# vkit-x/vkit

Hardware: AMD Instinct MI355X
Metric: Mpixels/s (2048^2 RGB, geo+photo chain) (higher is better)
Workload: dtype u8; 1 GPU; C3 fused chain: camera_cubic_curve remap (level 5) + gaussian_blur(sigma=1.0) + color_shift(37) + gaussion_noise(std=10.0, the numpy stream default_rng(5000 + i) drawn on the device inside every step), states built from the configs inside every step, 2048x2048x3 uint8, batch 256 per GPU; batch_per_gpu=256, image=2048x2048x3, noise_mode=tiles, states=built on the device from the configs inside every step (vkx_camera_states_dev), lanes=1

## Files before the change

vkit_amd/csrc/chain.hip:

```cpp
#include "vkx_internal.h"

#include <stdlib.h>
#include <algorithm>
#include <memory>
#include <unordered_map>
#include <vector>

static int chain_check_items(const vkx_chain_item *items, int n_items)
{
    for (int i = 0; i < n_items; i++) {
        const vkx_chain_item &it = items[i];
        VKX_REQUIRE(it.src && it.dst && it.src_vertices && it.dst_vertices, "NULL plane in chain item");
        VKX_REQUIRE(it.sh > 0 && it.sw > 0 && it.dh > 0 && it.dw > 0, "bad shape in chain item");
        VKX_REQUIRE_PITCH(it.src_stride, (ptrdiff_t)it.sw * 3, it.sh);
        VKX_REQUIRE_PITCH(it.dst_stride, (ptrdiff_t)it.dw * 3, it.dh);
        if (it.noise && !it.noise_tiled) VKX_REQUIRE_PITCH(it.noise_stride_el, (ptrdiff_t)it.dw * 3, it.dh);
        VKX_REQUIRE_DISJOINT(it.src, it.sh, it.src_stride, (size_t)it.sw * 3, it.dst, it.dh, it.dst_stride, (size_t)it.dw * 3);
        if (it.streak_enabled) {
            VKX_REQUIRE(it.streak_thickness + it.streak_gap > 0, "streak thickness + gap must be positive");
            if (it.streak_alpha < 0.0 || it.streak_alpha > 1.0) {
                vkx_set_error("alpha=%g is invalid.", it.streak_alpha);
                return VKX_ERR_INVALID;
            }
        }
// ... 13 lines not shown
    }
    static const bool staged_only = vkx_env_on("VKX_CHAIN_STAGED", 0);
    if (!staged_only) {
        const int frc = vkx_chain_fused_try(ctx, items, n_items);
        if (frc != VKX_ERR_UNSUPPORTED) return frc;
    }
    if (int mrc = vkx_chain_consume_lattices_mark(ctx)) return mrc;
    for (int k = 0; k < 2; k++) {
        int rc = vkx_scratch_reserve(ctx, &ctx->chain[k], max_plane);
        if (rc) return rc;
    }
    for (int i = 0; i < n_items; i++) {
        const vkx_chain_item &it = items[i];
        const bool blur = it.blur_ksize > 1;
        const bool hue = it.hue_enabled != 0;
        const bool noise = it.noise != nullptr;
        const int stages_after_remap = (blur ? 1 : 0) + (hue ? 1 : 0) + (noise ? 1 : 0);
        const ptrdiff_t tmp_stride = (ptrdiff_t)it.dw * 3;
        int remaining = stages_after_remap;
        int flip = 0;
        auto next_out = [&](uint8_t *&out, ptrdiff_t &stride) {
            if (remaining == 0) { out = it.dst; stride = it.dst_stride; }
            else { out = (uint8_t *)ctx->chain[flip].ptr; stride = tmp_stride; flip ^= 1; }
        };
        uint8_t *cur = nullptr;
        ptrdiff_t cur_stride = 0;
        next_out(cur, cur_stride);
        vkx_elem e;
        e.src = it.src; e.dst = cur; e.src_stride = it.src_stride; e.dst_stride = cur_stride; e.cn = 3; e.is_f32 = 0;
        int rc = vkx_grid_remap_dev(ctx, &e, 1, it.sh, it.sw, it.src_vertices, it.dst_vertices, it.rows, it.cols, it.dh,
                                    it.dw);
        if (rc) return rc;
        if (blur) {
            remaining--;
            uint8_t *out; ptrdiff_t ostride;
            next_out(out, ostride);
            rc = vkx_gaussian_blur_u8_dev(ctx, cur, it.dh, it.dw, 3, cur_stride, it.blur_ksize, it.blur_sigma, out, ostride);
            if (rc) return rc;
            cur = out; cur_stride = ostride;
        }
        if (hue) {
            remaining--;
            uint8_t *out; ptrdiff_t ostride;
            next_out(out, ostride);
            rc = vkx_color_shift_rgb_dev(ctx, cur, it.dh, it.dw, cur_stride, it.hue_delta, out, ostride);
            if (rc) return rc;
            cur = out; cur_stride = ostride;
        }
        if (noise) {
            remaining--;
            uint8_t *out; ptrdiff_t ostride;
            next_out(out, ostride);
            const int16_t *plane = it.noise;
            ptrdiff_t plane_stride = it.noise_stride_el;
            if (it.noise_tiled) {
                const long long n = (long long)it.dh * it.dw * 3;
                if ((rc = vkx_scratch_reserve(ctx, &ctx->chain[2], (size_t)n * 2))) return rc;
                if ((rc = vkx_np_tiles_expand_dev(ctx, it.noise, n, (int16_t *)ctx->chain[2].ptr))) return rc;
                plane = (const int16_t *)ctx->chain[2].ptr;
                plane_stride = (ptrdiff_t)it.dw * 3;
            }
            rc = vkx_add_noise_i16_dev(ctx, cur, it.dh, it.dw, 3, cur_stride, plane, plane_stride, out, ostride);
            if (rc) return rc;
            cur = out; cur_stride = ostride;
        }
        if (it.streak_enabled) {
            rc = vkx_line_streak_u8_dev(ctx, it.dst, it.dh, it.dw, 3, it.dst_stride, it.streak_thickness, it.streak_gap,
                                        it.streak_dash_thickness, it.streak_dash_gap, it.streak_color, it.streak_alpha,
                                        it.streak_enable_vert, it.streak_enable_hori);
            if (rc) return rc;
        }
    }
    return VKX_OK;
}

VKX_EXPORT int vkx_chain_rgb_batch_np_dev(vkx_ctx *ctx, const vkx_chain_item *items, int n_items, const vkx_np_job *jobs, int n_jobs,
                                          vkx_np_result *results_host)
{
    VKX_REQUIRE(ctx != nullptr, "ctx is NULL");
    VKX_REQUIRE(n_items >= 0 && (n_items == 0 || items), "bad item list");
    if (n_jobs <= 0) return vkx_chain_rgb_batch_dev(ctx, items, n_items);
    int rc = vkx_np_jobs_check(jobs, n_jobs, results_host);
    if (rc) return rc;
    if ((rc = chain_check_items(items, n_items))) return rc;
    std::unordered_map<const void *, int> item_of;
    for (int i = 0; i < n_items; i++)
        if (items[i].noise && items[i].noise_tiled) item_of[(const void *)items[i].noise] = i;
    bool pipelined = (jobs[0].kind & 0xff) == VKX_NP_NORMAL_TILES;
    std::vector<int> job_item((size_t)n_jobs, -1);
    for (int k = 0; k < n_jobs && pipelined; k++) {
        auto it = item_of.find(jobs[k].dst);
        if (it == item_of.end() || (k > 0 && it->second <= job_item[k - 1])) pipelined = false;
        else job_item[k] = it->second;
    }
    static const bool staged_only = vkx_env_on("VKX_CHAIN_STAGED", 0);
    static const int chunks_env = vkx_env_int("VKX_CHAIN_CHUNKS", 0);
    const int want_chunks = chunks_env > 0 ? chunks_env : 2;
    vkx_chain_plan *raw = nullptr;
    if (pipelined && !staged_only) {
        rc = vkx_chain_plan_build(ctx, items, n_items, &raw);
        if (rc && rc != VKX_ERR_UNSUPPORTED) return rc;
    }
    if (!raw) {
        if ((rc = vkx_chain_consume_lattices_mark(ctx))) return rc;
        if ((rc = vkx_np_draw_batch_dev(ctx, jobs, n_jobs, results_host))) return rc;
        return vkx_chain_rgb_batch_dev(ctx, items, n_items);
    }
    std::unique_ptr<vkx_chain_plan, void (*)(vkx_chain_plan *)> plan(raw, vkx_chain_plan_free);
    const int n_chunks = std::max(1, std::min(want_chunks, n_jobs / 8));
    struct Chunk { int job0, njobs, item0, nitems; vkx_np_chunk *np; hipEvent_t posted; };
    std::vector<Chunk> chunks((size_t)n_chunks);
    for (int c = 0; c < n_chunks; c++) {
        Chunk &ch = chunks[c];
        ch.job0 = (int)((long long)n_jobs * c / n_chunks);
        ch.njobs = (int)((long long)n_jobs * (c + 1) / n_chunks) - ch.job0;
        ch.item0 = c == 0 ? 0 : job_item[ch.job0];
        ch.np = nullptr; ch.posted = nullptr;
    }
    for (int c = 0; c < n_chunks; c++) chunks[c].nitems = (c + 1 < n_chunks ? chunks[c + 1].item0 : n_items) - chunks[c].item0;
    struct Cleanup {
        std::vector<Chunk> &chunks;
        ~Cleanup() { for (Chunk &ch : chunks) { if (ch.np) vkx_np_chunk_free(ch.np); if (ch.posted) (void)hipEventDestroy(ch.posted); } }
    } cleanup{chunks};

    vkx_device_guard guard(ctx);
    hipStream_t main_stream = ctx->stream;
    const char *fail_env = getenv("VKX_DEBUG_FAIL_CHUNK");
    const int fail_chunk = fail_env && fail_env[0] ? atoi(fail_env) : -1;
    auto schedule = [&]() -> int {
        int rc = VKX_OK;
        hipStream_t aux = vkx_stream_by_id(ctx, VKX_STREAM_COPY_IN, &rc);
        if (rc) return rc;
        hipEvent_t setup_done = nullptr;
        if ((rc = vkx_chain_plan_setup_aside(ctx, raw, &setup_done))) return rc;
        if (setup_done) VKX_HIP(hipStreamWaitEvent(aux, setup_done, 0));
        for (int c = 0; c < n_chunks; c++) {
            Chunk &ch = chunks[c];
            if (c >= 2) VKX_HIP(hipStreamWaitEvent(main_stream, chunks[c - 2].posted, 0));
            if ((rc = vkx_np_chunk_begin(ctx, jobs + ch.job0, ch.njobs, results_host + ch.job0, c & 1, &ch.np))) return rc;
            if ((rc = vkx_stream_order(ctx, aux, main_stream))) return rc;
            ctx->stream = aux;
            rc = vkx_np_chunk_finish(ctx, ch.np);
            if (!rc) rc = vkx_chain_plan_noise_rows(ctx, raw, ch.item0, ch.nitems);
            ctx->stream = main_stream;
            if (rc) return rc;
            VKX_HIP(hipEventCreateWithFlags(&ch.posted, hipEventDisableTiming));
            VKX_HIP(hipEventRecord(ch.posted, aux));
            if (c == fail_chunk) {
                vkx_set_error("injected failure in chunk %d (VKX_DEBUG_FAIL_CHUNK)", c);
                return VKX_ERR_INVALID;
            }
        }
        if (setup_done) VKX_HIP(hipStreamWaitEvent(main_stream, setup_done, 0));
        for (int c = 0; c < n_chunks; c++) {
            Chunk &ch = chunks[c];
            VKX_HIP(hipStreamWaitEvent(main_stream, ch.posted, 0));
            if ((rc = vkx_chain_plan_tiles(ctx, raw, ch.item0, ch.nitems))) return rc;
        }
        return vkx_chain_mark_done(ctx, main_stream);
    };
    rc = schedule();
    if (rc) vkx_ctx_join_streams(ctx, main_stream);
    return rc;
}
```

vkit_amd/csrc/fused.hip:

```cpp
#include "vkx_internal.h"
#include "vkx_cell.h"
#include "vkx_color.h"

#include <float.h>
#include <memory>
#include <stdlib.h>
#include <string.h>

namespace {

constexpr int W = 64;
constexpr int RMAX = 3;
constexpr int NLDSCELL = 64;
#ifndef VKX_FUSED_NWAVES
#define VKX_FUSED_NWAVES 8
#endif
constexpr int NWAVES = VKX_FUSED_NWAVES;
constexpr int NTHREADS = 64 * NWAVES;
constexpr int ROWS_PER_WAVE = 8;
constexpr int WH = NWAVES * ROWS_PER_WAVE;
__host__ __device__ constexpr int tile_side(int R) { return (W - 2 * R) & ~3; }
__host__ __device__ constexpr int tile_height(int R) { return WH == W ? tile_side(R) : WH - 2 * R; }
#ifndef VKX_FUSED_CGROUP
#define VKX_FUSED_CGROUP 2
// ... 784 lines not shown
    const uint32_t g4 = (uint32_t)((ocx >> 2) * 12 + (ocx & 3) * 4);
    const uint32_t k3 = grouped ? g4 : (uint32_t)(ocx * 3);
    const bool nlane = ocol && !(grouped && (ocx & 3) == 3);
    constexpr bool every_lane = INTERIOR;
    const uint32_t k3n = (every_lane && !nlane) ? 0u : k3;
    const uint32_t k3b = k3n << 1;
    long long prow = (long long)(y0 + wave) * (long long)nstride + (long long)x0 * 3;
    const long long pstep = (long long)NWAVES * (long long)nstride;
    if (noise) {
#pragma unroll
        for (int i = 0; i < ROWS_PER_WAVE; i++) {
            const int cy = wave + NWAVES * i;
            const long long prow_i = prow;
            prow += pstep;
            if (!row_live(i, cy)) continue;
            const uint32_t rx = (uint32_t)__builtin_amdgcn_readlane((int)nrow.x, i);
            const uint32_t sd = (uint32_t)__builtin_amdgcn_readlane((int)nrow.y, i) | never;
            const gbytes_t rowb = nbase + 2 * (tiled ? (long long)rx : prow_i);
            uint32_t off = k3b;
            if ((sd & 0xffffu) < 3u * W) {
                asm volatile("" ::: "memory");
                off += k3n >= (sd & 0xffffu) ? (uint32_t)((int)sd >> 16) << 1 : 0u;
            }
            const gbytes_t np_ = rowb + (size_t)off;
            if (!every_lane) { nzA[i] = 0; nzB[i] = 0; }
            if (every_lane || nlane) {
                if (grouped) {
                    const unsigned long long v = *(const u64_u1 VKX_GLOBAL *)np_;
                    nzA[i] = (uint32_t)v;
                    nzB[i] = (uint32_t)(v >> 32);
                } else {
                    nzA[i] = *(const u32_u1 VKX_GLOBAL *)np_;
                    nzB[i] = *(const u16_u1 VKX_GLOBAL *)(np_ + 4);
                }
            }
        }
    }
    uint32_t wpair[RMAX + 1];
#pragma unroll
    for (int q = 0; q <= RMAX; q++) {
        const uint32_t e0 = 2 * q < K ? kq[2 * q < 2 * RMAX + 1 ? 2 * q : 0] : 0u, e1 = 2 * q + 1 < K ? kq[2 * q + 1 < 2 * RMAX + 1 ? 2 * q + 1 : 0] : 0u;
        const uint32_t o0 = (q > 0 && 2 * q - 1 < K) ? kq[q > 0 ? 2 * q - 1 : 0] : 0u, o1 = 2 * q < K ? kq[2 * q < 2 * RMAX + 1 ? 2 * q : 0] : 0u;
        wpair[q] = (wave & 1) ? (o0 | (o1 << 16)) : (e0 | (e1 << 16));
    }
    const int right4 = min(lane + 1, 63) << 2;
    const uint32_t dcol4 = (uint32_t)(x0 * 3) + g4;
    const bool streak_on = STREAK && ite.streak_on != 0;
    const int sxm = streak_on ? (x0 + ocx) % ite.streak_step : 0;
    const int sxd = streak_on ? (x0 + ocx) % ite.streak_dash_step : 0;
    uint32_t epx = 0;
    if constexpr (EMPTY) {
        int er = src[0], eg = src[1], eb = src[2];
        if (hue_on) hue_shift_px(lut->sdiv, lut->hdiv, hue_delta, er, eg, eb);
        epx = (uint32_t)er | ((uint32_t)eg << 8) | ((uint32_t)eb << 16);
    }
#pragma unroll
    for (int i = 0; i < ROWS_PER_WAVE; i++) {
        const int cy = wave + NWAVES * i;
        if (!row_live(i, cy)) continue;
        const int gy = y0 + cy;
        uint32_t P = epx;
        if constexpr (!EMPTY) {
            if (R > 0) {
                int r, g, b;
                if constexpr (INTERIOR && RC > 0) {
                    const uint32_t *pl = own + (cy & ~1) * P_ + lane;
                    uint32_t ar = 32768u, ag = 32768u, ab = 32768u;
#pragma unroll
                    for (int q = 0; q <= RC; q++) {
                        ar = dot2_u16_ks(wpair[q], pl[q * kPairPitch], ar);
                        ag = dot2_u16_ks(wpair[q], pl[q * kPairPitch + 64], ag);
                        ab = dot2_u16_ks(wpair[q], pl[q * kPairPitch + 128], ab);
                    }
                    r = (int)(ar >> 16); g = (int)(ag >> 16); b = (int)(ab >> 16);
                } else {
                    uint32_t a0 = 0, a1 = 0, a2 = 0;
#pragma unroll
                    for (int j = 0; j < 2 * RMAX + 1; j++) {
                        if (j < K) {
                            const int yy = INTERIOR ? cy + j : vkd::reflect101(gy + j - R, dh) - wy0;
                            const uint16_t *h16 = (const uint16_t *)(own + (yy & ~1) * P_ + lane) + (yy & 1);
                            a0 += __umul24(kq[j], (uint32_t)h16[0]);
                            a1 += __umul24(kq[j], (uint32_t)h16[128]);
                            a2 += __umul24(kq[j], (uint32_t)h16[256]);
                        }
                    }
                    r = (int)((a0 + 32768u) >> 16); g = (int)((a1 + 32768u) >> 16); b = (int)((a2 + 32768u) >> 16);
                }
                if (phase_limit == 20) {
                    const int yy = INTERIOR ? cy + R : vkd::reflect101(gy, dh) - wy0;
                    const uint16_t *h16 = (const uint16_t *)(own + (yy & ~1) * P_ + lane) + (yy & 1);
                    r = h16[0] >> 8; g = h16[128] >> 8; b = h16[256] >> 8;
                }
                if (hue_on) P = vkd::hue_shift_packed(lsdiv, lhdiv, lsel, hue_delta, r, g, b);
                else P = (uint32_t)r | ((uint32_t)g << 8) | ((uint32_t)b << 16);
            } else {
                P = own[(cy + R) * P_ + lane];
                if (hue_on) P = vkd::hue_shift_packed(lsdiv, lhdiv, lsel, hue_delta, (int)(P & 0xff), (int)((P >> 8) & 0xff),
                                                      (int)((P >> 16) & 0xff));
            }
        }
        if ((STREAK || !INTERIOR) && ((noise && !grouped) || (STREAK && streak_on))) {
            int r = (int)(P & 0xff), g = (int)((P >> 8) & 0xff), b = (int)((P >> 16) & 0xff);
            if (noise) {
                r = vkd::clamp_u8((int)(int16_t)(r + (int)(nzA[i] & 0xffff)));
                g = vkd::clamp_u8((int)(int16_t)(g + (int)(nzA[i] >> 16)));
                b = vkd::clamp_u8((int)(int16_t)(b + (int)(nzB[i] & 0xffff)));
            }
            if (STREAK && streak_on) {
                const int ym = gy % ite.streak_step, yd = gy % ite.streak_dash_step;
                bool mv = ite.streak_vert && sxm < ite.streak_thickness;
                bool mh = ite.streak_hori && ym < ite.streak_thickness;
                if (ite.streak_dash) {
                    if (yd < ite.streak_dash_gap) mv = false;
                    if (sxd < ite.streak_dash_gap) mh = false;
                }
                const float w1 = ite.streak_alpha, w0 = 1.0f - w1;
                int *ch[3] = {&r, &g, &b};
#pragma unroll
                for (int c = 0; c < 3; c++) {
                    int v = *ch[c];
                    const int col = ite.streak_color[c];
                    if (mv) { const float t0 = w0 * (float)v, t1 = w1 * (float)col; v = ite.streak_copy ? col : (int)(uint8_t)(t0 + t1); }
                    if (mh) { const float t0 = w0 * (float)v, t1 = w1 * (float)col; v = ite.streak_copy ? col : (int)(uint8_t)(t0 + t1); }
                    *ch[c] = v;
                }
            }
            P = (uint32_t)r | ((uint32_t)g << 8) | ((uint32_t)b << 16);
        }
        const uint32_t Pn = (uint32_t)__builtin_amdgcn_ds_bpermute(right4, (int)P);
        gdst_t drow = dst + (ptrdiff_t)gy * dstride + (ptrdiff_t)x0 * 3;
        if (ocol) {
            const int m = ocx & 3;
            if (INTERIOR || ocx < full4) {
                if (m < 3) {
                    uint32_t wv = (P >> (8 * m)) | (Pn << (24 - 8 * m));
                    if (!STREAK && noise) wv = add_noise_u8x4(wv, nzA[i], nzB[i]);
                    const uint32_t off = (uint32_t)gy * (uint32_t)dstride + dcol4;
                    *(u32_u1 VKX_GLOBAL *)(dst + (size_t)off) = wv;
                }
            } else {
                gdst_t d = drow + ocx * 3;
                d[0] = (uint8_t)P; d[1] = (uint8_t)(P >> 8); d[2] = (uint8_t)(P >> 16);
            }
        }
    }
}

template <bool STREAK>
__global__ void __launch_bounds__(NTHREADS, VKX_FUSED_WAVES_PER_EU) k_chain_fused(const ItemDev *__restrict__ items,
                                                          const vkc::CellC *__restrict__ cells,
                                                          const TileBin *__restrict__ bins, int bin_slots,
                                                          int *__restrict__ over_count, int2 *__restrict__ over_list, int over_slots,
                                                          const HsvLut *__restrict__ lut, int phase_limit)
{
    const ItemDev &it = items[blockIdx.y];
    const int rw = it.rect_w;
    const int nrect = rw * it.rect_h;
    const int per = (nrect + 7) >> 3;
    const int run = (int)((blockIdx.x + blockIdx.y) & 7), pos = (int)(blockIdx.x >> 3);
    const int rl = run * per + pos;
    if (pos >= per || rl >= nrect) return;
    if (phase_limit == 10) return;
    const int ry = __builtin_amdgcn_readfirstlane(div_small(rl, rw, __builtin_amdgcn_rcpf((float)rw)));
    const int tx = it.rect_x0 + rl - ry * rw, ty = it.rect_y0 + ry;
    const int tl = ty * it.tiles_x + tx;
    const TileBin bin = bins[(size_t)blockIdx.y * bin_slots + tl];
    const int nc = bin.rmax1 > 0 ? max(0, bin.rmax1 - bin.rmin) * max(0, bin.cmax1 - bin.cmin) : 0;
#ifdef VKX_FUSED_CENSUS
    (void)nc;
    chain_tile<1, STREAK, VKX_FUSED_CENSUS>(it, tx, ty, cells, bin, lut, phase_limit);
    return;
#endif
    if (nc == 0) chain_tile<2, STREAK>(it, tx, ty, cells, bin, lut, phase_limit);
    else if (nc <= NLDSCELL && phase_limit != 3) {
        switch (it.R) {
        case 0: chain_tile<1, STREAK, 0>(it, tx, ty, cells, bin, lut, phase_limit); break;
        case 1: chain_tile<1, STREAK, 1>(it, tx, ty, cells, bin, lut, phase_limit); break;
        case 2: chain_tile<1, STREAK, 2>(it, tx, ty, cells, bin, lut, phase_limit); break;
        default: chain_tile<1, STREAK, 3>(it, tx, ty, cells, bin, lut, phase_limit); break;
        }
    } else if (threadIdx.x == 0) {
        const int k = atomicAdd(over_count, 1);
        if (k < over_slots) over_list[k] = make_int2((int)blockIdx.y, tl);
    }
}

template <bool STREAK>
__global__ void __launch_bounds__(NTHREADS, VKX_FUSED_WAVES_PER_EU) k_chain_fused_rim(const ItemDev *__restrict__ items,
                                                          const vkc::CellC *__restrict__ cells,
                                                          const TileBin *__restrict__ bins, int bin_slots,
                                                          const HsvLut *__restrict__ lut, int phase_limit)
{
    if (phase_limit == 10) return;
    const ItemDev &it = items[blockIdx.y];
    const int tiles_x = it.tiles_x, rw = it.rect_w, rh = it.rect_h;
    const int nrim = tiles_x * it.tiles_y - rw * rh;
    const int per = (nrim + 7) >> 3;
    const int run = (int)((blockIdx.x + blockIdx.y) & 7), pos = (int)(blockIdx.x >> 3);
    const int q = run * per + pos;
    if (pos >= per || q >= nrim) return;
    int tl;
    const int top = it.rect_y0 * tiles_x, bottom = (it.tiles_y - it.rect_y0 - rh) * tiles_x;
    if (rw * rh == 0 || q < top) tl = q;
    else if (q < top + bottom) tl = q - top + (it.rect_y0 + rh) * tiles_x;
    else {
        const int m = q - top - bottom, side = tiles_x - rw;
        const int r = __builtin_amdgcn_readfirstlane(div_small(m, side, __builtin_amdgcn_rcpf((float)side)));
        const int c = m - r * side;
        tl = (it.rect_y0 + r) * tiles_x + (c < it.rect_x0 ? c : c + rw);
    }
    const TileBin bin = bins[(size_t)blockIdx.y * bin_slots + tl];
    const int ty = __builtin_amdgcn_readfirstlane(div_small(tl, tiles_x, __builtin_amdgcn_rcpf((float)tiles_x)));
    const int tx = tl - ty * tiles_x;
    const int nc = bin.rmax1 > 0 ? max(0, bin.rmax1 - bin.rmin) * max(0, bin.cmax1 - bin.cmin) : 0;
    if (nc == 0) chain_tile<2, STREAK>(it, tx, ty, cells, bin, lut, phase_limit);
    else {
        switch (it.R) {
        case 0: chain_tile<0, STREAK, 0>(it, tx, ty, cells, bin, lut, phase_limit); break;
        case 1: chain_tile<0, STREAK, 1>(it, tx, ty, cells, bin, lut, phase_limit); break;
        case 2: chain_tile<0, STREAK, 2>(it, tx, ty, cells, bin, lut, phase_limit); break;
        default: chain_tile<0, STREAK, 3>(it, tx, ty, cells, bin, lut, phase_limit); break;
        }
    }
}

constexpr int kOverGrid = 512;
template <bool STREAK>
__global__ void __launch_bounds__(NTHREADS, 4) k_chain_fused_over(const ItemDev *__restrict__ items,
                                                          const vkc::CellC *__restrict__ cells,
                                                          const TileBin *__restrict__ bins, int bin_slots,
                                                          const int *__restrict__ over_count, const int2 *__restrict__ over_list,
                                                          int over_slots, const HsvLut *__restrict__ lut, int phase_limit)
{
    const int n_over = min(*over_count, over_slots);
    if ((int)blockIdx.x >= n_over || phase_limit == 10) return;
    for (int k = (int)blockIdx.x; k < n_over; k += (int)gridDim.x) {
        const int2 e = over_list[k];
        const int img = __builtin_amdgcn_readfirstlane(e.x), tl = __builtin_amdgcn_readfirstlane(e.y);
        const ItemDev &it = items[img];
        const TileBin bin = bins[(size_t)img * bin_slots + tl];
        const int tiles_x = __builtin_amdgcn_readfirstlane(it.tiles_x);
        const int ty = __builtin_amdgcn_readfirstlane(div_small(tl, tiles_x, __builtin_amdgcn_rcpf((float)tiles_x)));
        chain_tile<0, STREAK>(it, tl - ty * tiles_x, ty, cells, bin, lut, phase_limit);
        __syncthreads();
    }
}

template <bool STREAK>
__global__ void __launch_bounds__(NTHREADS, VKX_FUSED_WAVES_PER_EU) k_chain_fused_whole(const ItemDev *__restrict__ items,
                                                          const vkc::CellC *__restrict__ cells,
                                                          const TileBin *__restrict__ bins,
                                                          const HsvLut *__restrict__ lut, int phase_limit)
{
    const int slots = gridDim.x;
    const ItemDev &it = items[blockIdx.y];
    const int ntiles = it.tiles_x * it.tiles_y;
    const int per = (ntiles + 7) >> 3;
    const int run = (int)((blockIdx.x + blockIdx.y) & 7), pos = (int)(blockIdx.x >> 3);
    const int tl = run * per + pos;
    if (pos >= per || tl >= ntiles) return;
    if (phase_limit == 10) return;
    const int tile_id = (int)blockIdx.y * slots + tl;
    const TileBin bin = bins[tile_id];
    const int ty = __builtin_amdgcn_readfirstlane(div_small(tl, it.tiles_x, __builtin_amdgcn_rcpf((float)it.tiles_x)));
    const int tx = tl - ty * it.tiles_x;
    const int Tw = tile_side(it.R), Th = tile_height(it.R);
    const int wx0 = tx * Tw - it.R, wy0 = ty * Th - it.R;
    const int nc = bin.rmax1 > 0 ? max(0, bin.rmax1 - bin.rmin) * max(0, bin.cmax1 - bin.cmin) : 0;
    const bool interior = wx0 >= 0 && wy0 >= 0 && wx0 + W <= it.dw && wy0 + WH <= it.dh && nc <= NLDSCELL && phase_limit != 3;
    if (nc == 0) chain_tile<2, STREAK>(it, tx, ty, cells, bin, lut, phase_limit);
    else if (interior) {
        switch (it.R) {
        case 0: chain_tile<1, STREAK, 0>(it, tx, ty, cells, bin, lut, phase_limit); break;
        case 1: chain_tile<1, STREAK, 1>(it, tx, ty, cells, bin, lut, phase_limit); break;
        case 2: chain_tile<1, STREAK, 2>(it, tx, ty, cells, bin, lut, phase_limit); break;
        default: chain_tile<1, STREAK, 3>(it, tx, ty, cells, bin, lut, phase_limit); break;
        }
    } else {
        switch (it.R) {
        case 0: chain_tile<0, STREAK, 0>(it, tx, ty, cells, bin, lut, phase_limit); break;
        case 1: chain_tile<0, STREAK, 1>(it, tx, ty, cells, bin, lut, phase_limit); break;
        case 2: chain_tile<0, STREAK, 2>(it, tx, ty, cells, bin, lut, phase_limit); break;
        default: chain_tile<0, STREAK, 3>(it, tx, ty, cells, bin, lut, phase_limit); break;
        }
    }
}

__global__ void __launch_bounds__(NTHREADS, 8) k_tile_remap(const ItemDev *__restrict__ items,
                                                           const vkc::CellC *__restrict__ cells,
                                                           const TileBin *__restrict__ bins, const ElemPack pack)
{
    const int slots = gridDim.x;
    const ItemDev &it = items[blockIdx.y];
    const int ntiles = it.tiles_x * it.tiles_y;
    const int per = (ntiles + 7) >> 3;
    const int run = (int)((blockIdx.x + blockIdx.y) & 7), pos = (int)(blockIdx.x >> 3);
    const int tl = run * per + pos;
    if (pos >= per || tl >= ntiles) return;
    const int tile_id = (int)blockIdx.y * slots + tl;
    const TileBin bin = bins[tile_id];
    const int ty = __builtin_amdgcn_readfirstlane(div_small(tl, it.tiles_x, __builtin_amdgcn_rcpf((float)it.tiles_x)));
    const int tx = tl - ty * it.tiles_x;
    chain_tile<3>(it, tx, ty, cells, bin, nullptr, 0, &pack);
}

__global__ void __launch_bounds__(256) k_chain_noise_rows(const ItemDev *__restrict__ items)
{
    typedef uint32_t u32x2 __attribute__((ext_vector_type(2)));
    const ItemDev &it = items[blockIdx.y];
    if (!it.noise_rows) return;
    const uint32_t k = blockIdx.x * 256u + threadIdx.x;
    if (k >= (uint32_t)it.dh * (uint32_t)it.tiles_x) return;
    const uint32_t y = k / (uint32_t)it.tiles_x, tx = k - y * (uint32_t)it.tiles_x;
    const u32x2 VKX_GLOBAL *tab = (const u32x2 VKX_GLOBAL *)it.noise_table;
    const uint32_t T = (uint32_t)it.noise_tiles, slot = (uint32_t)it.noise_slot;
    const uint32_t i0 = (y * (uint32_t)it.dw + tx * (uint32_t)tile_side(it.R)) * 3u;
    const uint32_t g = min((uint32_t)((float)i0 * it.noise_tiles_per_sample), T - 1);
    const uint32_t gb = g > 0 ? g - 1 : 0;
    const u32x2 e0 = tab[min(gb, T)], e1 = tab[min(gb + 1, T)], e2 = tab[min(gb + 2, T)], e3 = tab[min(gb + 3, T)];
    uint32_t t;
    u32x2 a, b;
    if (i0 >= e2.x) { t = gb + 2; a = e2; b = e3; }
    else if (i0 >= e1.x) { t = gb + 1; a = e1; b = e2; }
    else { t = gb; a = e0; b = e1; }
    while (a.x > i0 && t > 0) { t--; b = a; a = tab[t]; }
    while (b.x <= i0 && t + 1 < T) { t++; a = b; b = tab[t + 1]; }
    const uint32_t before = min(b.x - i0, 0xffffu), step = slot + b.y - a.y - (b.x - a.x);
    u32x2 rec;
    rec.x = t * slot + a.y + (i0 - a.x);
    rec.y = before | (step << 16);
    ((u32x2 VKX_GLOBAL *)it.noise_rows)[k] = rec;
}

__global__ void __launch_bounds__(256) k_chain_prologue(uint32_t *__restrict__ desc_dst, const uint32_t *__restrict__ desc_src,
                                                        unsigned n_words, TileBin *__restrict__ bins, unsigned nbins,
                                                        int *__restrict__ deferred, int *__restrict__ over_count, unsigned n_over)
{
    const unsigned i = blockIdx.x * 256 + threadIdx.x;
    if (i < n_words) desc_dst[i] = desc_src[i];
    if (i < nbins) bins[i] = TileBin{0x7f7f7f7f, 0x7f7f7f7f, 0, 0};
    if (i < n_over) over_count[i] = 0;
    if (i == 0) *deferred = 0;
}

}

struct vkx_chain_plan {
    std::vector<ItemDev> dev;
    std::vector<int> prefix;
    std::vector<long long> row_prefix;
    long long ncells = 0;
    int max_tiles = 0, slots = 0;
    int rect_slots = 0;
    bool elements = false, streak = false;
    const ItemDev *d_items = nullptr;
    const int *d_cell_prefix = nullptr;
    TileBin *bins = nullptr;
    vkc::CellC *cells = nullptr;
    int *deferred = nullptr;
    int *over_count = nullptr;
    int2 *over_list = nullptr;
    const HsvLut *lut = nullptr;
};

void vkx_chain_plan_free(vkx_chain_plan *p) { delete p; }
int vkx_chain_plan_items(const vkx_chain_plan *p) { return (int)p->dev.size(); }

int vkx_chain_plan_setup(vkx_ctx *ctx, vkx_chain_plan *p)
{
    const int n_items = (int)p->dev.size();
    int rc;
    vkx_scratch *s_cells = p->elements ? &ctx->cells : &ctx->chain_cells;
    vkx_scratch *s_bins = p->elements ? &ctx->owner : &ctx->chain_bins;
    vkx_scratch *s_misc = p->elements ? &ctx->misc : &ctx->chain_misc;
    const size_t cells_bytes = sizeof(vkc::CellC) * (size_t)p->ncells;
    if ((rc = vkx_scratch_reserve(ctx, s_cells, cells_bytes + sizeof(int) * ((size_t)p->ncells + 1)))) return rc;
    p->slots = ((p->max_tiles + 7) / 8) * 8;
    const size_t nbins = (size_t)p->slots * n_items;
    if (n_items > 65535) return VKX_ERR_UNSUPPORTED;
    const size_t over_ints = p->elements ? 0 : (size_t)n_items * (2 + 2 * (size_t)p->rect_slots);
    if ((rc = vkx_scratch_reserve(ctx, s_bins, sizeof(TileBin) * nbins + sizeof(int) * over_ints))) return rc;
    const size_t items_bytes = sizeof(ItemDev) * (size_t)n_items, prefix_bytes = sizeof(int) * p->prefix.size();
    vkx_tables tab(ctx);
    const size_t items_off = tab.add(items_bytes), prefix_off = tab.add(prefix_bytes), misc_bytes = tab.bytes;
    if ((rc = vkx_scratch_reserve(ctx, s_misc, misc_bytes))) return rc;
    if (!p->elements && (rc = vkx_hsv_tables(ctx, (const void **)&p->lut))) return rc;
    unsigned char *misc = (unsigned char *)s_misc->ptr;
    if ((rc = tab.take())) return rc;
    memcpy(tab.at<char>(items_off), p->dev.data(), items_bytes);
    memcpy(tab.at<char>(prefix_off), p->prefix.data(), prefix_bytes);
    p->d_items = (const ItemDev *)(misc + items_off);
    p->d_cell_prefix = (const int *)(misc + prefix_off);
    p->bins = (TileBin *)s_bins->ptr;
    p->over_count = (int *)(p->bins + nbins);
    p->over_list = (int2 *)(p->over_count + n_items + (n_items & 1));
    p->cells = (vkc::CellC *)s_cells->ptr;
    p->deferred = (int *)((unsigned char *)s_cells->ptr + cells_bytes);
    {
        const unsigned char *ring_dev = tab.mapped();
        if (!ring_dev) { vkx_set_error("%s: the descriptor ring is not mapped into the device's address space", __func__); return VKX_ERR_HIP; }
        const size_t n_words = (misc_bytes + 3) / 4;
        VKX_TIMED(ctx, "k_chain_prologue");
        k_chain_prologue<<<vkx_blocks(std::max(n_words, nbins), 256), 256, 0, ctx->stream>>>((uint32_t *)misc, (const uint32_t *)ring_dev,
                                                                                            (unsigned)n_words, p->bins, (unsigned)nbins, p->deferred,
                                                                                            p->over_count, p->elements ? 0u : (unsigned)n_items);
        VKX_LAUNCH_CHECK();
    }
    { VKX_TIMED(ctx, "k_chain_setup"); k_chain_setup<<<vkx_blocks((size_t)p->ncells, 256), 256, 0, ctx->stream>>>(p->d_items, p->d_cell_prefix, n_items, (int)p->ncells, p->slots, p->cells, p->bins, p->deferred); }
    VKX_LAUNCH_CHECK();
    { VKX_TIMED(ctx, "k_chain_setup_svd"); k_chain_setup_svd<<<128, 64, 0, ctx->stream>>>(p->d_items, p->d_cell_prefix, n_items, p->cells, p->deferred); }
    VKX_LAUNCH_CHECK();
    return VKX_OK;
}

int vkx_chain_plan_noise_rows(vkx_ctx *ctx, vkx_chain_plan *p, int first, int count)
{
    if (p->row_prefix.empty() || count <= 0) return VKX_OK;
    long long most = 0;
    for (int i = first; i < first + count; i++) most = std::max(most, p->row_prefix[i + 1] - p->row_prefix[i]);
    if (most <= 0) return VKX_OK;
    VKX_TIMED(ctx, "k_chain_noise_rows");
    k_chain_noise_rows<<<dim3(vkx_blocks((size_t)most, 256), count), 256, 0, ctx->stream>>>(p->d_items + first);
    VKX_LAUNCH_CHECK();
    return VKX_OK;
}

int vkx_chain_plan_tiles(vkx_ctx *ctx, vkx_chain_plan *p, int first, int count)
{
    if (count <= 0) return VKX_OK;
    static const int phase_limit = vkx_env_int("VKX_FUSED_PHASES", 0);
    const ItemDev *items = p->d_items + first;
    const TileBin *bins = p->bins + (size_t)first * p->slots;
    if (p->elements) {
        const dim3 grid(p->slots, count);
        VKX_TIMED(ctx, "k_tile_remap");
        ElemPack pack;
        memset(&pack, 0, sizeof(pack));
        pack.n = p->dev[first].n_elems;
        for (int e = 0; e < 4; e++) pack.el[e] = p->dev[first].el[e];
        k_tile_remap<<<grid, NTHREADS, kFusedLds, ctx->stream>>>(items, p->cells, bins, pack);
    } else {
        int most_rect = 0, most_rim = 0;
        long long all_rect = 0, all_tiles = 0;
        for (int i = first; i < first + count; i++) {
            const ItemDev &d = p->dev[i];
            most_rect = std::max(most_rect, d.rect_w * d.rect_h);
            all_rect += d.rect_w * d.rect_h;
            all_tiles += (long long)d.tiles_x * d.tiles_y;
            most_rim = std::max(most_rim, d.tiles_x * d.tiles_y - d.rect_w * d.rect_h);
        }
        int *over_count = p->over_count + first;
        int2 *over_list = p->over_list + (size_t)first * p->rect_slots;
        const int over_slots = (int)std::min<long long>((long long)count * p->rect_slots, INT_MAX);
        VKX_TIMED_MAJOR(ctx, "k_chain_fused");
        constexpr long long kSplitMinTiles = 65536;
        const int split_env = vkx_env_on("VKX_CHAIN_SPLIT", -1);
        if (split_env >= 0 ? split_env == 0 : all_tiles < kSplitMinTiles) {
            const dim3 grid(p->slots, count);
            if (p->streak) k_chain_fused_whole<true><<<grid, NTHREADS, kFusedLds, ctx->stream>>>(items, p->cells, bins, p->lut, phase_limit);
            else k_chain_fused_whole<false><<<grid, NTHREADS, kFusedLds, ctx->stream>>>(items, p->cells, bins, p->lut, phase_limit);
            VKX_LAUNCH_CHECK();
            return VKX_OK;
        }
        if (most_rect > 0) {
            const dim3 grid_rect((most_rect + 7) / 8 * 8, count);
            if (p->streak) k_chain_fused<true><<<grid_rect, NTHREADS, kFusedLds, ctx->stream>>>(items, p->cells, bins, p->slots, over_count, over_list, over_slots, p->lut, phase_limit);
            else k_chain_fused<false><<<grid_rect, NTHREADS, kFusedLds, ctx->stream>>>(items, p->cells, bins, p->slots, over_count, over_list, over_slots, p->lut, phase_limit);
            VKX_LAUNCH_CHECK();
        }
        if (most_rim > 0) {
            const dim3 grid_rim((most_rim + 7) / 8 * 8, count);
            if (p->streak) k_chain_fused_rim<true><<<grid_rim, NTHREADS, kFusedLds, ctx->stream>>>(items, p->cells, bins, p->slots, p->lut, phase_limit);
            else k_chain_fused_rim<false><<<grid_rim, NTHREADS, kFusedLds, ctx->stream>>>(items, p->cells, bins, p->slots, p->lut, phase_limit);
            VKX_LAUNCH_CHECK();
        }
        if (most_rect > 0) {
            const dim3 grid_over((unsigned)std::min<long long>((all_rect + 1) / 2, kOverGrid));
            if (p->streak) k_chain_fused_over<true><<<grid_over, NTHREADS, kFusedLds, ctx->stream>>>(items, p->cells, bins, p->slots, over_count, over_list, over_slots, p->lut, phase_limit);
            else k_chain_fused_over<false><<<grid_over, NTHREADS, kFusedLds, ctx->stream>>>(items, p->cells, bins, p->slots, over_count, over_list, over_slots, p->lut, phase_limit);
        }
    }
    VKX_LAUNCH_CHECK();
    return VKX_OK;
}

int vkx_chain_plan_build(vkx_ctx *ctx, const vkx_chain_item *items, int n_items, vkx_chain_plan **out)
{
    *out = nullptr;
    if (n_items <= 0) return VKX_OK;
    std::unique_ptr<vkx_chain_plan> plan(new vkx_chain_plan());
    std::vector<ItemDev> &dev = plan->dev;
    dev.resize(n_items);
    plan->prefix.resize((size_t)n_items + 1);
    int *cell_prefix = plan->prefix.data();
    std::vector<long long> &row_prefix = plan->row_prefix;
    row_prefix.assign((size_t)n_items + 1, 0);
    long long tiles = 0, ncells = 0;
    int max_tiles = 0, max_rect = 0;
    for (int i = 0; i < n_items; i++) {
        const vkx_chain_item &it = items[i];
        if (it.blur_ksize > 2 * RMAX + 1 || (it.blur_ksize > 1 && (it.blur_ksize & 1) == 0)) return VKX_ERR_UNSUPPORTED;
        if (it.sh > 32767 || it.sw > 32767 || it.dh > 32767 || it.dw > 32767) return VKX_ERR_UNSUPPORTED;
        if (it.rows < 2 || it.cols < 2) return VKX_ERR_UNSUPPORTED;
        if (it.blur_ksize > 1 && (it.dh == 1 || it.dw == 1)) return VKX_ERR_UNSUPPORTED;
        ItemDev &d = dev[i];
        memset(&d, 0, sizeof(d));
        d.src = it.src; d.dst = it.dst; d.noise = it.noise; d.sv = it.src_vertices; d.dv = it.dst_vertices;
        d.sstride = it.src_stride; d.dstride = it.dst_stride; d.nstride = it.noise_stride_el;
        d.noise_table = nullptr; d.noise_tiled = 0; d.noise_tiles = 0; d.noise_slot = 0; d.noise_tiles_per_sample = 0.f;
        d.noise_rows = nullptr;
        if (it.noise && it.noise_tiled) {
            const long long n = (long long)it.dh * it.dw * 3;
            if (n > 0x7fffffffLL) return VKX_ERR_UNSUPPORTED;
            const vkx_np_tiles_shape shape = vkx_np_tiles_shape_of(n);
            if (shape.n_tiles * shape.slot_elems > 0xffffffffLL) return VKX_ERR_UNSUPPORTED;
            d.noise = (const int16_t *)((const unsigned char *)it.noise + shape.slots_offset);
            d.noise_table = (const uint2 *)((const unsigned char *)it.noise + shape.table_offset);
            d.noise_tiled = 1; d.noise_tiles = (int)shape.n_tiles; d.noise_slot = shape.slot_elems;
            d.noise_tiles_per_sample = (float)(1.0 / shape.samples_per_tile);
        }
        d.sh = it.sh; d.sw = it.sw; d.dh = it.dh; d.dw = it.dw; d.rows = it.rows; d.cols = it.cols;
        d.R = it.blur_ksize > 1 ? it.blur_ksize / 2 : 0;
        const int Tw = tile_side(d.R), Th = tile_height(d.R);
        d.tiles_x = (it.dw + Tw - 1) / Tw; d.tiles_y = (it.dh + Th - 1) / Th;
        const TileRect rect = interior_rect(it.dw, it.dh, d.R);
        if (!rect.empty()) { d.rect_x0 = rect.x0; d.rect_y0 = rect.y0; d.rect_w = rect.x1 - rect.x0 + 1; d.rect_h = rect.y1 - rect.y0 + 1; }
        max_rect = std::max(max_rect, d.rect_w * d.rect_h);
        d.cell_base = (int)ncells;
        d.hue_on = it.hue_enabled; d.hue_delta = it.hue_delta;
        d.streak_on = it.streak_enabled && it.streak_alpha != 0.0 && (it.streak_enable_vert || it.streak_enable_hori);
        if (it.streak_enabled) {
            if (it.streak_thickness + it.streak_gap <= 0) return VKX_ERR_UNSUPPORTED;
            d.streak_thickness = it.streak_thickness;
            d.streak_step = it.streak_thickness + it.streak_gap;
            d.streak_dash = it.streak_dash_thickness > 0 && it.streak_dash_gap > 0;
            d.streak_dash_step = d.streak_dash ? it.streak_dash_thickness + it.streak_dash_gap : 1;
            d.streak_dash_gap = it.streak_dash_gap;
            d.streak_vert = it.streak_enable_vert; d.streak_hori = it.streak_enable_hori;
            d.streak_copy = it.streak_alpha == 1.0;
            d.streak_alpha = (float)it.streak_alpha;
            for (int c = 0; c < 3; c++) d.streak_color[c] = it.streak_color[c];
        }
        for (int k = 0; k < 8; k++) d.kq[k] = 0;
        if (d.R > 0 && vkx_gaussian_kernel_q8_host(it.blur_ksize, it.blur_sigma, d.kq)) return VKX_ERR_UNSUPPORTED;
        for (int k = 0; k < d.R; k++)
            if (d.kq[k] != d.kq[2 * d.R - k]) return VKX_ERR_UNSUPPORTED;
        if (it.src_stride <= 0 || it.src_stride >= (1 << 24) || (long long)it.sh * it.src_stride + 8 > 0xffffffffLL) return VKX_ERR_UNSUPPORTED;
        if (it.dst_stride <= 0 || (long long)it.dh * it.dst_stride > 0xffffffffLL) return VKX_ERR_UNSUPPORTED;
        cell_prefix[i] = (int)ncells;
        row_prefix[i + 1] = row_prefix[i] + (d.noise_tiled ? (long long)it.dh * d.tiles_x : 0);
        tiles += (long long)d.tiles_x * d.tiles_y;
        if (d.tiles_x * d.tiles_y > max_tiles) max_tiles = d.tiles_x * d.tiles_y;
        ncells += (long long)(it.rows - 1) * (it.cols - 1);
        if (tiles > 0x3fffffff || ncells > 0x3fffffff) return VKX_ERR_UNSUPPORTED;
        plan->streak = plan->streak || d.streak_on != 0;
    }
    cell_prefix[n_items] = (int)ncells;
    if (n_items > 65535) return VKX_ERR_UNSUPPORTED;
    if (row_prefix[n_items] > 0) {
        int rc = vkx_scratch_reserve(ctx, &ctx->noise_rows, (size_t)row_prefix[n_items] * sizeof(uint2));
        if (rc) return rc;
        for (int i = 0; i < n_items; i++)
            if (dev[i].noise_tiled) dev[i].noise_rows = (const uint2 *)ctx->noise_rows.ptr + row_prefix[i];
    } else {
        row_prefix.clear();
    }
    plan->ncells = ncells;
    plan->max_tiles = max_tiles;
    plan->rect_slots = (max_rect + 7) / 8 * 8;
    *out = plan.release();
    return VKX_OK;
}

int vkx_chain_plan_setup_aside(vkx_ctx *ctx, vkx_chain_plan *p, hipEvent_t *done)
{
    static const int aside_env = vkx_env_on("VKX_CHAIN_SETUP_ASIDE", -1);
    constexpr size_t kAsideMinItems = 16;
    const bool aside = aside_env >= 0 ? aside_env != 0 : p->dev.size() >= kAsideMinItems;
    *done = nullptr;
    if (!aside) {
        if (ctx->lattices_armed) {
            vkx_device_guard guard(ctx);
            VKX_HIP(hipStreamWaitEvent(ctx->stream, ctx->lattices_ready, 0));
            ctx->lattices_armed = false;
        }
        return vkx_chain_plan_setup(ctx, p);
    }
    int rc;
    hipStream_t main_stream = ctx->stream;
    hipStream_t side = vkx_stream_by_id(ctx, VKX_STREAM_COPY_OUT, &rc);
    if (rc) return rc;
    vkx_device_guard guard(ctx);
    if (ctx->lattices_armed) {
        VKX_HIP(hipStreamWaitEvent(side, ctx->lattices_ready, 0));
        ctx->lattices_armed = false;
    } else if ((rc = vkx_stream_order(ctx, side, main_stream))) return rc;
    if (ctx->chain_done) VKX_HIP(hipStreamWaitEvent(side, ctx->chain_done, 0));
    ctx->stream = side;
    rc = vkx_chain_plan_setup(ctx, p);
    ctx->stream = main_stream;
    if (rc) return rc;
    if (!ctx->chain_setup_done) VKX_HIP(hipEventCreateWithFlags(&ctx->chain_setup_done, hipEventDisableTiming));
    VKX_HIP(hipEventRecord(ctx->chain_setup_done, side));
    *done = ctx->chain_setup_done;
    return VKX_OK;
}

int vkx_chain_mark_done(vkx_ctx *ctx, hipStream_t stream)
{
    if (!ctx->chain_done) VKX_HIP(hipEventCreateWithFlags(&ctx->chain_done, hipEventDisableTiming));
    VKX_HIP(hipEventRecord(ctx->chain_done, stream));
    return VKX_OK;
}

int vkx_chain_fused_try(vkx_ctx *ctx, const vkx_chain_item *items, int n_items)
{
    vkx_chain_plan *raw = nullptr;
    int rc = vkx_chain_plan_build(ctx, items, n_items, &raw);
    if (rc || !raw) return rc;
    std::unique_ptr<vkx_chain_plan, void (*)(vkx_chain_plan *)> plan(raw, vkx_chain_plan_free);
    hipStream_t main_stream = ctx->stream;
    auto schedule = [&]() -> int {
        int rc;
        hipEvent_t setup_done = nullptr;
        if ((rc = vkx_chain_plan_setup_aside(ctx, raw, &setup_done))) return rc;
        if (setup_done) VKX_HIP(hipStreamWaitEvent(ctx->stream, setup_done, 0));
        if ((rc = vkx_chain_plan_noise_rows(ctx, raw, 0, n_items))) return rc;
        if ((rc = vkx_chain_plan_tiles(ctx, raw, 0, n_items))) return rc;
        vkx_device_guard guard(ctx);
        return vkx_chain_mark_done(ctx, ctx->stream);
    };
    rc = schedule();
    if (rc) vkx_ctx_join_streams(ctx, main_stream);
    return rc;
}

int vkx_tile_remap_try(vkx_ctx *ctx, const vkx_elem *elems, int n_elems, int sh, int sw, const int32_t *src_vertices,
// ... 36 lines not shown
```

vkit_amd/csrc/vkx_internal.h:

```cpp
#pragma once
#include <hip/hip_runtime.h>
#include <stdint.h>
#include <stddef.h>
#include <limits.h>
#include <stdlib.h>
#include <string>
#include <vector>

#include "../../include/vkx.h"

#define VKX_EXPORT extern "C" __attribute__((visibility("default")))

void vkx_set_error(const char *fmt, ...);

#define VKX_HIP(call)                                                                      \
    do {                                                                                   \
        hipError_t e__ = (call);                                                           \
        if (e__ != hipSuccess) {                                                           \
            vkx_set_error("%s failed: %s (%s:%d)", #call, hipGetErrorString(e__), __FILE__, \
                          __LINE__);                                                       \
            return VKX_ERR_HIP;                                                            \
        }                                                                                  \
    } while (0)

// ... 202 lines not shown
    return hipMemcpy2DAsync(dst, dst_pitch, src, src_pitch, row_bytes, rows, kind, stream);
}

static inline unsigned vkx_blocks(size_t n, unsigned per_block)
{
    size_t b = (n + per_block - 1) / per_block;
    return (unsigned)(b < 1 ? 1 : b);
}

namespace vkd {

__device__ __forceinline__ int cv_round(float v)
{
    if (!(fabsf(v) < 2147483648.f)) return INT_MIN;
    return __float2int_rn(v);
}
__device__ __forceinline__ int cv_round(double v)
{
    if (!(v >= -2147483648.5 && v < 2147483647.5)) return INT_MIN;
    return __double2int_rn(v);
}
__device__ __forceinline__ int reflect101(int p, int len)
{
    if ((unsigned)p < (unsigned)len) return p;
    if (len == 1) return 0;
    do {
        if (p < 0) p = -p;
        else p = 2 * (len - 1) - p;
    } while ((unsigned)p >= (unsigned)len);
    return p;
}
template <class Prefix>
__device__ __forceinline__ int last_at_most(int n, int t, Prefix prefix)
{
    int lo = 0, hi = n - 1;
    while (lo < hi) {
        const int mid = (lo + hi + 1) >> 1;
        if (prefix(mid) <= t) lo = mid; else hi = mid - 1;
    }
    return lo;
}
__device__ __forceinline__ int sat_short(int v) { return v < -32768 ? -32768 : (v > 32767 ? 32767 : v); }
__device__ __forceinline__ int clamp_u8(int v) { return v < 0 ? 0 : (v > 255 ? 255 : v); }

template <int CN, class Tap>
__device__ __forceinline__ void sample_taps_u8(Tap tap, int sh, int sw, int X, int Y, uint8_t *out)
{
    const int sx = sat_short(X >> 5), sy = sat_short(Y >> 5);
    const int fx = X & 31, fy = Y & 31;
    if (sx >= sw || sx + 1 < 0 || sy >= sh || sy + 1 < 0) {
#pragma unroll
        for (int k = 0; k < CN; k++) out[k] = 0;
        return;
    }
    const bool x0 = sx >= 0, x1 = sx + 1 < sw, y0 = sy >= 0, y1 = sy + 1 < sh;
    const int w00 = (32 - fy) * (32 - fx), w01 = (32 - fy) * fx, w10 = fy * (32 - fx), w11 = fy * fx;
#pragma unroll
    for (int k = 0; k < CN; k++) {
        const int v0 = (x0 && y0) ? tap(sy, sx, k) : 0;
        const int v1 = (x1 && y0) ? tap(sy, sx + 1, k) : 0;
        const int v2 = (x0 && y1) ? tap(sy + 1, sx, k) : 0;
        const int v3 = (x1 && y1) ? tap(sy + 1, sx + 1, k) : 0;
        out[k] = (uint8_t)((v0 * w00 + v1 * w01 + v2 * w10 + v3 * w11 + 512) >> 10);
    }
}
template <int CN, typename PTR = const uint8_t *>
__device__ __forceinline__ void sample_u8(PTR src, int sh, int sw, ptrdiff_t sstride, int X, int Y, uint8_t *out)
{
    sample_taps_u8<CN>([&](int y, int x, int k) { return (int)src[(ptrdiff_t)y * sstride + (ptrdiff_t)x * CN + k]; }, sh, sw, X, Y, out);
}

template <typename PTR = const float *>
__device__ __forceinline__ float sample_f32(PTR src, int sh, int sw, ptrdiff_t sstride_el, int X, int Y)
{
    const int sx = sat_short(X >> 5), sy = sat_short(Y >> 5);
    const int fx = X & 31, fy = Y & 31;
    if (sx >= sw || sx + 1 < 0 || sy >= sh || sy + 1 < 0) return 0.f;
    const bool x0 = sx >= 0, x1 = sx + 1 < sw, y0 = sy >= 0, y1 = sy + 1 < sh;
    const PTR r0 = src + (ptrdiff_t)sy * sstride_el + sx;
    const PTR r1 = r0 + sstride_el;
    const float ax = fx * (1.f / 32), ay = fy * (1.f / 32);
    const float bx = 1.f - ax, by = 1.f - ay;
    const float w0 = by * bx, w1 = by * ax, w2 = ay * bx, w3 = ay * ax;
    const float v0 = (x0 && y0) ? r0[0] : 0.f;
    const float v1 = (x1 && y0) ? r0[1] : 0.f;
    const float v2 = (x0 && y1) ? r1[0] : 0.f;
    const float v3 = (x1 && y1) ? r1[1] : 0.f;
    const float p0 = v0 * w0, p1 = v1 * w1, p2 = v2 * w2, p3 = v3 * w3;
    return ((p0 + p1) + p2) + p3;
}

struct CoordPerspective {
    static constexpr bool kTile2D = true;
    double m[9];
    int bw0;
    struct Column {};
    struct Rows {};
    __device__ __forceinline__ Column column(int) const { return Column(); }
    __device__ __forceinline__ Rows rows(int, int) const { return Rows(); }
    __device__ __forceinline__ void at(const Column &, const Rows &, int, int x, int y, int &X, int &Y) const { (*this)(x, y, X, Y); }
    __device__ __forceinline__ void operator()(int x, int y, int &X, int &Y) const
    {
        const int xb = (x / bw0) * bw0, x1 = x - xb;
        const double X0 = m[0] * xb + m[1] * y + m[2];
        const double Y0 = m[3] * xb + m[4] * y + m[5];
        const double W0 = m[6] * xb + m[7] * y + m[8];
        double W = W0 + m[6] * x1;
        W = W ? 32 / W : 0;
        const double fX = fmax((double)INT_MIN, fmin((double)INT_MAX, (X0 + m[0] * x1) * W));
        const double fY = fmax((double)INT_MIN, fmin((double)INT_MAX, (Y0 + m[3] * x1) * W));
        X = vkd::cv_round(fX);
        Y = vkd::cv_round(fY);
    }
};

__host__ __device__ inline CoordPerspective make_perspective(const double S[9], int dh, int dw)
{
    CoordPerspective c;
    auto at = [&](int r, int col) { return S[r * 3 + col]; };
    double d = at(0, 0) * (at(1, 1) * at(2, 2) - at(1, 2) * at(2, 1)) -
               at(0, 1) * (at(1, 0) * at(2, 2) - at(1, 2) * at(2, 0)) +
               at(0, 2) * (at(1, 0) * at(2, 1) - at(1, 1) * at(2, 0));
    if (d == 0.) {
        for (int i = 0; i < 9; i++) c.m[i] = 0;
    } else {
        d = 1. / d;
        c.m[0] = (at(1, 1) * at(2, 2) - at(1, 2) * at(2, 1)) * d;
        c.m[1] = (at(0, 2) * at(2, 1) - at(0, 1) * at(2, 2)) * d;
        c.m[2] = (at(0, 1) * at(1, 2) - at(0, 2) * at(1, 1)) * d;
        c.m[3] = (at(1, 2) * at(2, 0) - at(1, 0) * at(2, 2)) * d;
        c.m[4] = (at(0, 0) * at(2, 2) - at(0, 2) * at(2, 0)) * d;
        c.m[5] = (at(0, 2) * at(1, 0) - at(0, 0) * at(1, 2)) * d;
        c.m[6] = (at(1, 0) * at(2, 1) - at(1, 1) * at(2, 0)) * d;
        c.m[7] = (at(0, 1) * at(2, 0) - at(0, 0) * at(2, 1)) * d;
        c.m[8] = (at(0, 0) * at(1, 1) - at(0, 1) * at(1, 0)) * d;
    }
    const int BLOCK_SZ = 32;
    const int bh0 = BLOCK_SZ / 2 < dh ? BLOCK_SZ / 2 : (dh > 0 ? dh : 1);
    c.bw0 = BLOCK_SZ * BLOCK_SZ / bh0 < dw ? BLOCK_SZ * BLOCK_SZ / bh0 : (dw > 0 ? dw : 1);
    return c;
}

}

int vkx_hsv_tables(vkx_ctx *ctx, const void **out);
int vkx_gaussian_kernel_q8_host(int n, double sigma, uint16_t *kq);
int vkx_chain_fused_try(vkx_ctx *ctx, const vkx_chain_item *items, int n_items);
struct vkx_chain_plan;
int vkx_chain_plan_build(vkx_ctx *ctx, const vkx_chain_item *items, int n_items, vkx_chain_plan **out);
void vkx_chain_plan_free(vkx_chain_plan *p);
int vkx_chain_plan_setup_aside(vkx_ctx *ctx, vkx_chain_plan *p, hipEvent_t *done);
int vkx_chain_plan_noise_rows(vkx_ctx *ctx, vkx_chain_plan *p, int first, int count);
int vkx_chain_plan_tiles(vkx_ctx *ctx, vkx_chain_plan *p, int first, int count);
int vkx_chain_mark_done(vkx_ctx *ctx, hipStream_t stream);
struct vkx_np_chunk;
int vkx_np_jobs_check(const vkx_np_job *jobs, int n_jobs, const vkx_np_result *results_host);
int vkx_np_chunk_begin(vkx_ctx *ctx, const vkx_np_job *jobs, int n_jobs, vkx_np_result *results_host, int slot, vkx_np_chunk **out);
int vkx_np_chunk_finish(vkx_ctx *ctx, vkx_np_chunk *c);
void vkx_np_chunk_free(vkx_np_chunk *c);
int vkx_tile_remap_try(vkx_ctx *ctx, const vkx_elem *elems, int n_elems, int sh, int sw, const int32_t *src_vertices,
                       const int32_t *dst_vertices, int rows, int cols, int dh, int dw);
struct vkx_np_tiles_shape {
    long long n_tiles;
    int slot_elems;
    size_t table_offset, slots_offset, bytes;
    double samples_per_tile;
};
vkx_np_tiles_shape vkx_np_tiles_shape_of(long long n);
```

Baseline: 76760 Mpixels/s.

## Batch rim and overflow passes across chunks into one joined launch

When every chunk qualifies for the split path, each chunk now launches only the interior-rect kernel. The rim and overflow kernels then run once over all items after the last chunk, with overflow entries recorded under global image indices in a shared list. This replaces two launches per chunk with two launches in total, giving larger grids and fewer small tail launches. The trade-off is that rim and overflow work can no longer overlap with later chunks' noise preparation, and it all waits until the end.

```diff
diff --git a/vkit_amd/csrc/chain.hip b/vkit_amd/csrc/chain.hip
--- a/vkit_amd/csrc/chain.hip
+++ b/vkit_amd/csrc/chain.hip
@@ -189,11 +189,14 @@
             }
         }
         if (setup_done) VKX_HIP(hipStreamWaitEvent(main_stream, setup_done, 0));
+        bool joined = n_chunks > 1;
+        for (int c = 0; c < n_chunks && joined; c++) joined = vkx_chain_plan_ranges_split(raw, chunks[c].item0, chunks[c].nitems);
         for (int c = 0; c < n_chunks; c++) {
             Chunk &ch = chunks[c];
             VKX_HIP(hipStreamWaitEvent(main_stream, ch.posted, 0));
-            if ((rc = vkx_chain_plan_tiles(ctx, raw, ch.item0, ch.nitems))) return rc;
-        }
+            if ((rc = joined ? vkx_chain_plan_tiles_interior(ctx, raw, ch.item0, ch.nitems) : vkx_chain_plan_tiles(ctx, raw, ch.item0, ch.nitems))) return rc;
+        }
+        if (joined && (rc = vkx_chain_plan_tiles_rest(ctx, raw))) return rc;
         return vkx_chain_mark_done(ctx, main_stream);
     };
     rc = schedule();
diff --git a/vkit_amd/csrc/fused.hip b/vkit_amd/csrc/fused.hip
--- a/vkit_amd/csrc/fused.hip
+++ b/vkit_amd/csrc/fused.hip
@@ -960,7 +960,7 @@
                                                           const vkc::CellC *__restrict__ cells,
                                                           const TileBin *__restrict__ bins, int bin_slots,
                                                           int *__restrict__ over_count, int2 *__restrict__ over_list, int over_slots,
-                                                          const HsvLut *__restrict__ lut, int phase_limit)
+                                                          const HsvLut *__restrict__ lut, int phase_limit, int img_base)
 {
     const ItemDev &it = items[blockIdx.y];
     const int rw = it.rect_w;
@@ -990,7 +990,7 @@
         }
     } else if (threadIdx.x == 0) {
         const int k = atomicAdd(over_count, 1);
-        if (k < over_slots) over_list[k] = make_int2((int)blockIdx.y, tl);
+        if (k < over_slots) over_list[k] = make_int2((int)blockIdx.y + img_base, tl);
     }
 }
 
@@ -1234,7 +1234,14 @@
     return VKX_OK;
 }
 
-int vkx_chain_plan_tiles(vkx_ctx *ctx, vkx_chain_plan *p, int first, int count)
+static bool chain_split_wanted(long long tiles)
+{
+    constexpr long long kSplitMinTiles = 65536;
+    const int split_env = vkx_env_on("VKX_CHAIN_SPLIT", -1);
+    return split_env >= 0 ? split_env != 0 : tiles >= kSplitMinTiles;
+}
+
+static int chain_tiles(vkx_ctx *ctx, vkx_chain_plan *p, int first, int count, int parts, bool joined)
 {
     if (count <= 0) return VKX_OK;
     static const int phase_limit = vkx_env_int("VKX_FUSED_PHASES", 0);
@@ -1258,32 +1265,31 @@
             all_tiles += (long long)d.tiles_x * d.tiles_y;
             most_rim = std::max(most_rim, d.tiles_x * d.tiles_y - d.rect_w * d.rect_h);
         }
-        int *over_count = p->over_count + first;
-        int2 *over_list = p->over_list + (size_t)first * p->rect_slots;
-        const int over_slots = (int)std::min<long long>((long long)count * p->rect_slots, INT_MAX);
+        int *over_count = p->over_count + (joined ? 0 : first);
+        int2 *over_list = p->over_list + (size_t)(joined ? 0 : first) * p->rect_slots;
+        const int over_slots = (int)std::min<long long>((long long)(joined ? (int)p->dev.size() : count) * p->rect_slots, INT_MAX);
+        const int img_base = joined ? first : 0;
         VKX_TIMED_MAJOR(ctx, "k_chain_fused");
-        constexpr long long kSplitMinTiles = 65536;
-        const int split_env = vkx_env_on("VKX_CHAIN_SPLIT", -1);
-        if (split_env >= 0 ? split_env == 0 : all_tiles < kSplitMinTiles) {
+        if (!joined && !chain_split_wanted(all_tiles)) {
             const dim3 grid(p->slots, count);
             if (p->streak) k_chain_fused_whole<true><<<grid, NTHREADS, kFusedLds, ctx->stream>>>(items, p->cells, bins, p->lut, phase_limit);
             else k_chain_fused_whole<false><<<grid, NTHREADS, kFusedLds, ctx->stream>>>(items, p->cells, bins, p->lut, phase_limit);
             VKX_LAUNCH_CHECK();
             return VKX_OK;
         }
-        if (most_rect > 0) {
+        if (most_rect > 0 && (parts & 1)) {
             const dim3 grid_rect((most_rect + 7) / 8 * 8, count);
-            if (p->streak) k_chain_fused<true><<<grid_rect, NTHREADS, kFusedLds, ctx->stream>>>(items, p->cells, bins, p->slots, over_count, over_list, over_slots, p->lut, phase_limit);
-            else k_chain_fused<false><<<grid_rect, NTHREADS, kFusedLds, ctx->stream>>>(items, p->cells, bins, p->slots, over_count, over_list, over_slots, p->lut, phase_limit);
+            if (p->streak) k_chain_fused<true><<<grid_rect, NTHREADS, kFusedLds, ctx->stream>>>(items, p->cells, bins, p->slots, over_count, over_list, over_slots, p->lut, phase_limit, img_base);
+            else k_chain_fused<false><<<grid_rect, NTHREADS, kFusedLds, ctx->stream>>>(items, p->cells, bins, p->slots, over_count, over_list, over_slots, p->lut, phase_limit, img_base);
             VKX_LAUNCH_CHECK();
         }
-        if (most_rim > 0) {
+        if (most_rim > 0 && (parts & 2)) {
             const dim3 grid_rim((most_rim + 7) / 8 * 8, count);
             if (p->streak) k_chain_fused_rim<true><<<grid_rim, NTHREADS, kFusedLds, ctx->stream>>>(items, p->cells, bins, p->slots, p->lut, phase_limit);
             else k_chain_fused_rim<false><<<grid_rim, NTHREADS, kFusedLds, ctx->stream>>>(items, p->cells, bins, p->slots, p->lut, phase_limit);
             VKX_LAUNCH_CHECK();
         }
-        if (most_rect > 0) {
+        if (most_rect > 0 && (parts & 2)) {
             const dim3 grid_over((unsigned)std::min<long long>((all_rect + 1) / 2, kOverGrid));
             if (p->streak) k_chain_fused_over<true><<<grid_over, NTHREADS, kFusedLds, ctx->stream>>>(items, p->cells, bins, p->slots, over_count, over_list, over_slots, p->lut, phase_limit);
             else k_chain_fused_over<false><<<grid_over, NTHREADS, kFusedLds, ctx->stream>>>(items, p->cells, bins, p->slots, over_count, over_list, over_slots, p->lut, phase_limit);
@@ -1292,6 +1298,17 @@
     VKX_LAUNCH_CHECK();
     return VKX_OK;
 }
+
+int vkx_chain_plan_tiles(vkx_ctx *ctx, vkx_chain_plan *p, int first, int count) { return chain_tiles(ctx, p, first, count, 3, false); }
+
+bool vkx_chain_plan_ranges_split(const vkx_chain_plan *p, int first, int count)
+{
+    long long tiles = 0;
+    for (int i = first; i < first + count; i++) tiles += (long long)p->dev[i].tiles_x * p->dev[i].tiles_y;
+    return !p->elements && count > 0 && chain_split_wanted(tiles);
+}
+int vkx_chain_plan_tiles_interior(vkx_ctx *ctx, vkx_chain_plan *p, int first, int count) { return chain_tiles(ctx, p, first, count, 1, true); }
+int vkx_chain_plan_tiles_rest(vkx_ctx *ctx, vkx_chain_plan *p) { return chain_tiles(ctx, p, 0, (int)p->dev.size(), 2, true); }
 
 int vkx_chain_plan_build(vkx_ctx *ctx, const vkx_chain_item *items, int n_items, vkx_chain_plan **out)
 {
diff --git a/vkit_amd/csrc/vkx_internal.h b/vkit_amd/csrc/vkx_internal.h
--- a/vkit_amd/csrc/vkx_internal.h
+++ b/vkit_amd/csrc/vkx_internal.h
@@ -378,6 +378,9 @@
 int vkx_chain_plan_setup_aside(vkx_ctx *ctx, vkx_chain_plan *p, hipEvent_t *done);
 int vkx_chain_plan_noise_rows(vkx_ctx *ctx, vkx_chain_plan *p, int first, int count);
 int vkx_chain_plan_tiles(vkx_ctx *ctx, vkx_chain_plan *p, int first, int count);
+bool vkx_chain_plan_ranges_split(const vkx_chain_plan *p, int first, int count);
+int vkx_chain_plan_tiles_interior(vkx_ctx *ctx, vkx_chain_plan *p, int first, int count);
+int vkx_chain_plan_tiles_rest(vkx_ctx *ctx, vkx_chain_plan *p);
 int vkx_chain_mark_done(vkx_ctx *ctx, hipStream_t stream);
 struct vkx_np_chunk;
 int vkx_np_jobs_check(const vkx_np_job *jobs, int n_jobs, const vkx_np_result *results_host);
```

After: 77220 Mpixels/s, median of 6. About the same (+0.6%).
